# MerlinPCarson/WakeWord-Detection

Hardware: AMD Instinct MI355X
Metric: audio frames/sec (16 kHz, 40-mel, 10 ms hop) + FRR@0.5 FA/h (higher is better)
Workload: dtype f32; 1 GPU; CRNN forward, batch=256x1.5 s synthetic 16 kHz clips per GPU, PCM resident in HBM -> log-mel (fp64 FFT) -> 151x40 window -> encode+detect, fp32 MFMA; clips_per_gpu=256, samples_per_clip=24000, resident_input_batches_rotated=24, resident_input_bytes=294912000, pipelined_contexts=4, weights=reference tf_lite_models (shipped fp32 weights), parallelism=single GPU

## Files before the change

### wakeword-detection_amd/csrc/crnn.hip

```cpp
#include "stream_fe.h"
#include <algorithm>
#include <type_traits>

#include <cstdlib>

typedef float f32x4 __attribute__((ext_vector_type(4)));

struct win_addr {
  const int64_t *row;
  const int32_t *valid;
  int64_t row0;
  int hop;
  int valid_const;
  int64_t mel_rows;
};

__device__ __forceinline__ void window_span(const win_addr &wa, int w, int T, int64_t &row, int &valid) {
  if (wa.row && wa.valid) {
    const int64_t r = wa.row[w];
    const int v = wa.valid[w];
    row = r;
    valid = v;
  } else {
    row = wa.row ? wa.row[w] : wa.row0 + (int64_t)w * wa.hop;
// ... 132 lines not shown
  for (int ni = 0; ni < 2; ++ni) {
    const int gn = n0 + wc * 32 + ni * 16 + i16;
    const float bv = (gn < g.N) ? g.bias[gn] : 0.f;
#pragma unroll
    for (int r = 0; r < 4; ++r) {
      const int gm = m0 + wr * 16 + kk * 4 + r;
      if (gm < g.M && gn < g.N) g.C[(size_t)gm * g.N + gn] = acc[ni][r] + bv;
    }
  }
}

#define GR_H 32
#define GR_SEQ_LD 68
#define GR_GX_LD 196
#define GR_W1_LD 65

__device__ __forceinline__ float fast_sigmoid(float x) {
  return __builtin_amdgcn_rcpf(1.0f + __builtin_amdgcn_exp2f(-1.4426950408889634f * x));
}
__device__ __forceinline__ float fast_tanh(float x) {
  const float e = __builtin_amdgcn_exp2f(2.8853900817779268f * x);
  return __fmaf_rn(-2.0f, __builtin_amdgcn_rcpf(1.0f + e), 1.0f);
}
__device__ __forceinline__ float gru_candidate(float r, float hc, float xc) { return fast_tanh(__fmaf_rn(r, hc, xc)); }
__device__ __forceinline__ float gru_blend(float z, float h, float c) { return __fmaf_rn(z, h, __fmul_rn(__fsub_rn(1.0f, z), c)); }

__device__ __forceinline__ float swap_pair(float v) {
  return __int_as_float(__builtin_amdgcn_mov_dpp(__float_as_int(v), 0xB1, 0xF, 0xF, true));
}

typedef float f32x2 __attribute__((ext_vector_type(2)));

struct gru_w {
  f32x2 z[8], r[8], c[8];
  float bz, br, bc;
};

__device__ __forceinline__ void gru_load_w(gru_w &g, const float *wh, const float *bh, int dir, int unit, int half) {
  const float *base = wh + (size_t)dir * 3 * GR_H * GR_H;
#pragma unroll
  for (int q = 0; q < 4; ++q) {
    const float4 z = *(const float4 *)(base + (size_t)(0 * GR_H + unit) * GR_H + half * 16 + q * 4);
    const float4 r = *(const float4 *)(base + (size_t)(1 * GR_H + unit) * GR_H + half * 16 + q * 4);
    const float4 c = *(const float4 *)(base + (size_t)(2 * GR_H + unit) * GR_H + half * 16 + q * 4);
    g.z[2 * q] = (f32x2){z.x, z.y}; g.z[2 * q + 1] = (f32x2){z.z, z.w};
    g.r[2 * q] = (f32x2){r.x, r.y}; g.r[2 * q + 1] = (f32x2){r.z, r.w};
    g.c[2 * q] = (f32x2){c.x, c.y}; g.c[2 * q + 1] = (f32x2){c.z, c.w};
  }
  g.bz = half ? 0.f : bh[dir * 3 * GR_H + unit];
  g.br = half ? 0.f : bh[dir * 3 * GR_H + GR_H + unit];
  g.bc = half ? 0.f : bh[dir * 3 * GR_H + 2 * GR_H + unit];
}

template <bool PREFETCH>
__device__ __forceinline__ float gru_step(const gru_w &g, const float *hin, int half, float gz, float gr, float gc, float h_own,
                                          const float *gx_next, float &nz, float &nr, float &nc) {
  const float4 *hp = (const float4 *)(hin + half * 16);
  float4 hv[4];
  hv[0] = hp[0];
  __builtin_amdgcn_sched_barrier(0);
  hv[1] = hp[1];
  hv[2] = hp[2];
  hv[3] = hp[3];
  __builtin_amdgcn_sched_barrier(0);
  if (PREFETCH) {
    nz = gx_next[0];
    nr = gx_next[GR_H];
    nc = gx_next[2 * GR_H];
  }
  f32x2 az = {half ? 0.f : gz, g.bz}, ar = {half ? 0.f : gr, g.br}, ac = {0.f, g.bc};
  __builtin_amdgcn_sched_barrier(0);
#pragma unroll
  for (int q = 0; q < 4; ++q) {
    const f32x2 h0 = {hv[q].x, hv[q].y}, h1 = {hv[q].z, hv[q].w};
    az = __builtin_elementwise_fma(g.z[2 * q], h0, az); ar = __builtin_elementwise_fma(g.r[2 * q], h0, ar); ac = __builtin_elementwise_fma(g.c[2 * q], h0, ac);
    __builtin_amdgcn_sched_barrier(0);
    az = __builtin_elementwise_fma(g.z[2 * q + 1], h1, az); ar = __builtin_elementwise_fma(g.r[2 * q + 1], h1, ar); ac = __builtin_elementwise_fma(g.c[2 * q + 1], h1, ac);
    __builtin_amdgcn_sched_barrier(0);
  }
  float sz = az.x + az.y, sr = ar.x + ar.y, sc = ac.x + ac.y;
  sz += swap_pair(sz);
  sr += swap_pair(sr);
  sc += swap_pair(sc);
  const float z = fast_sigmoid(sz);
  const float r = fast_sigmoid(sr);
  return gru_blend(z, h_own, gru_candidate(r, sc, gc));
}

__device__ __forceinline__ void wsync_h() {
  asm volatile("" ::: "memory");
  __builtin_amdgcn_wave_barrier();
}

__device__ __forceinline__ void lds_barrier() {
  asm volatile("s_waitcnt lgkmcnt(0)\n\ts_barrier" ::: "memory");
}

__device__ __forceinline__ void wsync_g() {
  asm volatile("s_waitcnt lgkmcnt(0)" ::: "memory");
  __builtin_amdgcn_wave_barrier();
}

#define CLEAR_SEQ_H(seq1_, rows_, hb_, threads_)                                      \
  for (int i = tid; i < (rows_) * GR_SEQ_LD; i += (threads_)) (seq1_)[i] = 0.f;       \
  for (int i = tid; i < 2 * 2 * 2 * GR_H; i += (threads_)) (hb_)[i] = 0.f;

#define CV_LOAD_W(wreg_, wlast_, cb0_, cb1_, w4_, cbias_)                                            \
  _Pragma("unroll") for (int kb = 0; kb < CV_KB; ++kb)                                               \
    _Pragma("unroll") for (int n = 0; n < 2; ++n)                                                    \
      wreg_[kb][n] = *(const float4 *)((w4_) + ((size_t)(kb * 4 + kk) * 32 + n * 16 + j) * 4);       \
  _Pragma("unroll") for (int n = 0; n < 2; ++n)                                                      \
    wlast_[n] = (w4_)[((size_t)CV_QL * 32 + n * 16 + j) * 4 + kk];                                   \
  cb0_ = (cbias_)[j];                                                                                \
  cb1_ = (cbias_)[16 + j];
struct cv_a {
  float4 q[CV_KB];
  float last;
};
#define CV_LOAD_A(av_, abase_)                                                                       \
  _Pragma("unroll") for (int kb = 0; kb < CV_KB; ++kb) {                                             \
    const int k4 = kb * 16 + kk * 4;                                                                 \
    const int kf = k4 / CV_KT, kt = k4 - kf * CV_KT;                                                 \
    av_.q[kb] = *(const float4 *)((abase_) + kf * CV_LDT + kt);                                      \
  }                                                                                                  \
  av_.last = (abase_)[(CV_QL * 4 / CV_KT) * CV_LDT + CV_QL * 4 % CV_KT + kk];
#define CV_MFMA_KB(av_, kb_)                                                                         \
  acc0 = __builtin_amdgcn_mfma_f32_16x16x4f32(av_.q[kb_].x, wreg[kb_][0].x, acc0, 0, 0, 0);           \
  acc1 = __builtin_amdgcn_mfma_f32_16x16x4f32(av_.q[kb_].x, wreg[kb_][1].x, acc1, 0, 0, 0);           \
  acc0 = __builtin_amdgcn_mfma_f32_16x16x4f32(av_.q[kb_].y, wreg[kb_][0].y, acc0, 0, 0, 0);           \
  acc1 = __builtin_amdgcn_mfma_f32_16x16x4f32(av_.q[kb_].y, wreg[kb_][1].y, acc1, 0, 0, 0);           \
  acc0 = __builtin_amdgcn_mfma_f32_16x16x4f32(av_.q[kb_].z, wreg[kb_][0].z, acc0, 0, 0, 0);           \
  acc1 = __builtin_amdgcn_mfma_f32_16x16x4f32(av_.q[kb_].z, wreg[kb_][1].z, acc1, 0, 0, 0);           \
  acc0 = __builtin_amdgcn_mfma_f32_16x16x4f32(av_.q[kb_].w, wreg[kb_][0].w, acc0, 0, 0, 0);           \
  acc1 = __builtin_amdgcn_mfma_f32_16x16x4f32(av_.q[kb_].w, wreg[kb_][1].w, acc1, 0, 0, 0);
#define CV_MFMA_LAST(av_)                                                                            \
  acc0 = __builtin_amdgcn_mfma_f32_16x16x4f32(av_.last, wlast[0], acc0, 0, 0, 0);                     \
  acc1 = __builtin_amdgcn_mfma_f32_16x16x4f32(av_.last, wlast[1], acc1, 0, 0, 0);
#define CV_TILE_LOOP(NT_, ...)                                                                       \
  {                                                                                                  \
    cv_a av[2];                                                                                      \
    load_a(av[0], 0);                                                                                \
    _Pragma("unroll") for (int i = 0; i < NT_; ++i) {                                                \
      if (i + 1 < NT_) load_a(av[(i + 1) & 1], i + 1);                                               \
      __builtin_amdgcn_sched_barrier(0);                                                             \
      f32x4 acc0 = {cb0, cb0, cb0, cb0}, acc1 = {cb1, cb1, cb1, cb1};                                \
      CV_MFMA_KB(av[i & 1], 0) CV_MFMA_KB(av[i & 1], 1) CV_MFMA_KB(av[i & 1], 2)                     \
      __builtin_amdgcn_sched_barrier(0);                                                             \
      __VA_ARGS__                                                                                    \
      __builtin_amdgcn_sched_barrier(0);                                                             \
      CV_MFMA_KB(av[i & 1], 3) CV_MFMA_KB(av[i & 1], 4) CV_MFMA_KB(av[i & 1], 5) CV_MFMA_LAST(av[i & 1]) \
      prev0 = acc0;                                                                                  \
      prev1 = acc1;                                                                                  \
    }                                                                                                \
  }

#define PJ_KS_BYTES (4 * 192 * 16)
typedef const __attribute__((address_space(1))) char *pj_gptr;
typedef const __attribute__((address_space(1))) f32x4 *pj_gptr4;
__device__ __forceinline__ float4 pj_w_ld(pj_gptr4 p) {
  const f32x4 v = *p;
  return make_float4(v.x, v.y, v.z, v.w);
}
#define PJ_W_LANE(wx1s_)                                                                             \
  const pj_gptr wb_0 = (pj_gptr)(wx1s_);                                                             \
  unsigned wb_lane = (unsigned)((kk * 192 + wave * 48 + j) * 16);
#define PJ_W_KSTEP(wk_, ks_)                                                                         \
  pj_gptr wk_ = wb_0 + (size_t)(ks_) * PJ_KS_BYTES;                                                  \
  asm("" : "+s"(wk_));                                                                               \
// ... 24 lines not shown
    if (ks + 1 < 40) { __VA_ARGS__ }                                                                 \
    __builtin_amdgcn_sched_barrier(0);                                                               \
    const float4 *b = bq[ks % DEPTH_];                                                               \
    G16_(x) G3_(x) G16_(y) G3_(y) G16_(z) G3_(z) G16_(w) G3_(w)                                      \
    __builtin_amdgcn_sched_barrier(0);                                                               \
  }
#define PJ_REM_ROWS(rem_, bv_, ...)                                                                  \
  _Pragma("unroll") for (int i = 0; i < 3; ++i) {                                                    \
    float s3 = rem_[i];                                                                              \
    s3 += __shfl_xor(s3, 16);                                                                        \
    s3 += __shfl_xor(s3, 32);                                                                        \
    if (kk == 0) {                                                                                   \
      const float v = s3 + bv_;                                                                      \
      __VA_ARGS__                                                                                    \
    }                                                                                                \
  }

#define CF_THREADS 256
#define CF_FLD 648
#define CF_IMG_FLOATS (CV_ROWS * CV_LDT)
#define CF_FEAT_FLOATS (CV_OT * CF_FLD)
#define CF_SMEM_BYTES ((CF_IMG_FLOATS + CF_FEAT_FLOATS) * 4)
#define CF_NO_ROW (-0x40000000)
#define CF_FUSED_FEAT_ROWS 13
#define CF_FUSED_SMEM_BYTES ((CF_IMG_FLOATS + CF_FUSED_FEAT_ROWS * CF_FLD) * 4)
#define CF_ALIAS_ROWS0 24
#define CF_ALIAS_REM (CF_ALIAS_ROWS0 + 3 * CF_FLD)
static_assert((((CF_ALIAS_ROWS0 - CF_IMG_FLOATS) / 4 - 2 * 13) % 16 + 16) % 16 == 0 && CF_IMG_FLOATS % 4 == 0, "aliased rows off their bank slots");
static_assert(CV_OT - 16 == 3 && 16 - CF_FUSED_FEAT_ROWS == 3 && CF_ALIAS_REM + 20 * 96 <= 20 * GR_GX_LD ,
              "the aliased rows must lie under gx");
#define CF_GX 0
#define CF_SEQ (20 * GR_GX_LD)
#define CF_HB (CF_SEQ + 32 * GR_SEQ_LD)
#define CF_ENC (CF_HB + 2 * 2 * 2 * GR_H)
#define CF_HID (CF_ENC + 2 * GR_H)
#define CF_W2S (CF_HID + 2 * GR_H)
static_assert(CF_W2S + 8 * 64 <= CF_IMG_FLOATS, "post-conv LDS layout exceeds the image region");
static_assert(64 * GR_W1_LD <= CF_FEAT_FLOATS && 16 * 192 * 4 <= CF_FEAT_FLOATS, "feat region too small for its later tenants");
static_assert(64 * GR_W1_LD <= CF_FUSED_FEAT_ROWS * CF_FLD, "fused kernel's feat region too small for the head's first layer");

struct fused_args {
  const float *mel;
  win_addr wa;
  const float *w4;
  const float *cbias;
  const float *wx1s;
  const float *bx1;
  const float *wh1, *bh1;
  const float *wx2s;
  const float *bx2, *wh2, *bh2, *w1, *b1, *w2, *b2;
  float *enc;
  float *out;
  int T, NOUT, HEAD;
  long long *stamps;
  float *gx_out;
  const unsigned short *cwb;
  const unsigned short *wx1b;
  ww_tick_tag tag;
};

template <bool SEQ>
__device__ __forceinline__ float cf_recurrence(const gru_w &g, const float *gxs, float *hd, float *seq1, int dir, int unit, int half) {
  constexpr int H = GR_H, OT = CV_OT;
  const float *gxl = gxs + dir * 3 * H + unit;
  float h_own = 0.f;
  int t = dir ? OT - 1 : 0;
  float gz = gxl[t * GR_GX_LD], gr = gxl[t * GR_GX_LD + H], gc = gxl[t * GR_GX_LD + 2 * H];
  for (int s = 0; s < OT; ++s) {
    const int cur = s & 1;
    const int tn = dir ? (t > 0 ? t - 1 : 0) : (t + 1 < OT ? t + 1 : OT - 1);
    float nz, nr, nc;
    h_own = gru_step<true>(g, hd + cur * H, half, gz, gr, gc, h_own, gxl + tn * GR_GX_LD, nz, nr, nc);
    if (half == 0) {
      hd[(cur ^ 1) * H + unit] = h_own;
      if (SEQ) seq1[t * GR_SEQ_LD + dir * H + unit] = h_own;
    }
    wsync_h();
    gz = nz; gr = nr; gc = nc;
    t = tn;
  }
  return h_own;
}

#define CF_ROUND_L2(av_, rv_, b_, e_)                                                                  \
  acc[0] = __builtin_amdgcn_mfma_f32_16x16x4f32(av_.e_, b_[0].e_, acc[0], 0, 0, 0);                     \
  acc[1] = __builtin_amdgcn_mfma_f32_16x16x4f32(av_.e_, b_[1].e_, acc[1], 0, 0, 0);                     \
  acc[2] = __builtin_amdgcn_mfma_f32_16x16x4f32(av_.e_, b_[2].e_, acc[2], 0, 0, 0);                     \
  rem[0] = __builtin_amdgcn_mfma_f32_16x16x4f32(rv_.e_, b_[0].e_, rem[0], 0, 0, 0);                     \
  rem[1] = __builtin_amdgcn_mfma_f32_16x16x4f32(rv_.e_, b_[1].e_, rem[1], 0, 0, 0);                     \
  rem[2] = __builtin_amdgcn_mfma_f32_16x16x4f32(rv_.e_, b_[2].e_, rem[2], 0, 0, 0);

#define L2_LOAD_W(bq_, wx2s_, nt0_)                                                                  \
  _Pragma("unroll") for (int kb = 0; kb < 4; ++kb)                                                   \
    _Pragma("unroll") for (int n = 0; n < 3; ++n)                                                    \
      bq_[kb][n] = *(const float4 *)((wx2s_) + ((size_t)(kb * 4 + kk) * 192 + ((nt0_) + n) * 16 + j) * 4);
#define L2_LOAD_BIAS(bb_, bx2_, nt0_) \
  _Pragma("unroll") for (int n = 0; n < 3; ++n) bb_[n] = (bx2_)[((nt0_) + n) * 16 + j];
#define L2_PROJECT(bq_, bb_, rrow_, nt0_, ...)                                                       \
  {                                                                                                  \
    f32x4 acc[3] = {{0.f, 0.f, 0.f, 0.f}, {0.f, 0.f, 0.f, 0.f}, {0.f, 0.f, 0.f, 0.f}};               \
    f32x4 rem[3] = {{0.f, 0.f, 0.f, 0.f}, {0.f, 0.f, 0.f, 0.f}, {0.f, 0.f, 0.f, 0.f}};               \
    _Pragma("unroll") for (int kb = 0; kb < 4; ++kb) {                                               \
      const float4 av = *(const float4 *)(&seq1[j * GR_SEQ_LD + kb * 16 + kk * 4]);                  \
      const float4 rv = *(const float4 *)(&seq1[(rrow_) * GR_SEQ_LD + kb * 16 + kk * 4]);            \
      const float4 *b = bq_[kb];                                                                     \
      CF_ROUND_L2(av, rv, b, x) CF_ROUND_L2(av, rv, b, y) CF_ROUND_L2(av, rv, b, z) CF_ROUND_L2(av, rv, b, w) \
    }                                                                                                \
    __VA_ARGS__                                                                                      \
    _Pragma("unroll") for (int n = 0; n < 3; ++n) {                                                  \
      const int col = ((nt0_) + n) * 16 + j;                                                         \
      const float bb = bb_[n];                                                                       \
      _Pragma("unroll") for (int r = 0; r < 4; ++r) gxs[(kk * 4 + r) * GR_GX_LD + col] = acc[n][r] + bb; \
      if (kk == 0) {                                                                                 \
        _Pragma("unroll") for (int r = 0; r < 3; ++r) gxs[(16 + r) * GR_GX_LD + col] = rem[n][r] + bb; \
      }                                                                                              \
    }                                                                                                \
  }

__device__ __forceinline__ void cf_phases_d_to_g(const fused_args &a, float *img, float *feat, const gru_w &g, int w) {
  constexpr int H = GR_H;
  const int tid = threadIdx.x, lane = tid & 63, wave = tid >> 6;
  const int j = lane & 15, kk = lane >> 4;
  const int unit = lane >> 1, half = lane & 1, dir = wave & 1;
  float *gxs = img + CF_GX, *seq1 = img + CF_SEQ, *hb = img + CF_HB, *encs = img + CF_ENC, *hid = img + CF_HID, *w2s = img + CF_W2S;
  float4 bq2[4][3];
  L2_LOAD_W(bq2, a.wx2s, wave * 3)
  if (wave < 2) {
    __builtin_amdgcn_s_setprio(3);
    cf_recurrence<true>(g, gxs, hb + dir * 2 * H, seq1, dir, unit, half);
    __builtin_amdgcn_s_setprio(0);
  }
  __syncthreads();

  {
    float bb2[3];
    L2_LOAD_BIAS(bb2, a.bx2, wave * 3)
    __builtin_amdgcn_sched_barrier(0);
    L2_PROJECT(bq2, bb2, 16 + j, wave * 3, )
  }
  __syncthreads();

  float *w1s = feat;
  if (wave >= 2) {
    __builtin_amdgcn_s_setprio(3);
    const float h_last = cf_recurrence<false>(g, gxs, hb + (2 + dir) * 2 * H, nullptr, dir, unit, half);
    __builtin_amdgcn_s_setprio(0);
    if (half == 0) {
      encs[dir * H + unit] = h_last;
      if (a.enc) a.enc[(size_t)w * 2 * H + dir * H + unit] = h_last;
    }
  } else {
    for (int i = tid; i < 64 * 64; i += 128) w1s[(i >> 6) * GR_W1_LD + (i & 63)] = a.w1[i];
    for (int i = tid; i < a.NOUT * 64; i += 128) w2s[i] = a.w2[i];
  }
  __syncthreads();

  if (wave == 0) {
    const float b1v = a.b1[lane], b2v = a.b2[lane < a.NOUT ? lane : 0];
    __builtin_amdgcn_sched_barrier(0);
    float acc = 0.f;
#pragma unroll 16
    for (int k = 0; k < 2 * H; ++k) acc = fmaf(w1s[lane * GR_W1_LD + k], encs[k], acc);
    hid[lane] = fmaxf(acc + b1v, 0.f);
    wsync_g();
    float y = 0.f;
    if (lane < a.NOUT) {
      for (int k = 0; k < 2 * H; ++k) y = fmaf(w2s[lane * 64 + k], hid[k], y);
      y += b2v;
    }
    const float p = head_activation(y, lane, a.NOUT, a.HEAD);
    if (a.tag.slots) {
      if (lane == a.tag.pidx) tick_tag_store(a.tag, w, p);
    } else if (lane < a.NOUT) {
      a.out[(size_t)w * a.NOUT + lane] = p;
    }
  }
}

#define CF_STAMP(i_) \
  if (FRONT_ONLY && a.stamps && lane == 0) a.stamps[((size_t)blockIdx.x * 4 + wave) * 10 + (i_)] = __builtin_amdgcn_s_memtime();
__device__ __forceinline__ void cf_set_move(fused_args &a, long long off) {
  ww_set_move(a.w4, off); ww_set_move(a.cbias, off); ww_set_move(a.wx1s, off); ww_set_move(a.bx1, off);
  ww_set_move(a.wh1, off); ww_set_move(a.bh1, off); ww_set_move(a.wx2s, off); ww_set_move(a.bx2, off);
  ww_set_move(a.wh2, off); ww_set_move(a.bh2, off); ww_set_move(a.w1, off); ww_set_move(a.b1, off);
  ww_set_move(a.w2, off); ww_set_move(a.b2, off); ww_set_move(a.cwb, off); ww_set_move(a.wx1b, off);
}
template <bool FRONT_ONLY, bool SET = false>
__global__ __launch_bounds__(CF_THREADS, 2) void crnn_fused_kernel(fused_args a, ww_set_ref set) {
  if constexpr (SET) cf_set_move(a, ww_set_offset(set, blockIdx.x));
  extern __shared__ __align__(16) float cf_smem[];
  float *img = cf_smem, *feat = cf_smem + CF_IMG_FLOATS;
  constexpr int H = GR_H, OT = CV_OT;
  const int tid = threadIdx.x, lane = tid & 63, wave = tid >> 6;
  const int j = lane & 15, kk = lane >> 4;
  const int w = blockIdx.x;
  CF_STAMP(0)
  int64_t row;
  int valid;
  window_span(a.wa, w, a.T, row, valid);

  float4 wreg[CV_KB][2];
  float wlast[2], cb0, cb1;
  CV_LOAD_W(wreg, wlast, cb0, cb1, a.w4, a.cbias)

  int a_off[6], o_off[6][4];
  {
    constexpr int MAXV = 6;
    const float *src = a.mel + row * CV_NMEL;
    const int n = valid * CV_NMEL;
    const bool al16 = ((((uintptr_t)src) & 15) == 0);
    float4 stage[MAXV];
    if (n > 0)
      stage_loads(al16, [&](auto al) {
        constexpr bool AL = decltype(al)::value;
#pragma unroll
        for (int q = 0; q < MAXV; ++q) {
          const int i = (q * CF_THREADS + tid) * 4;
          stage[q] = ld_mel4<AL>(src + (i < n ? i : n - 4), true);
        }
      });
    LDS_CLEAR16(img, CF_IMG_FLOATS / 4, CF_THREADS)
// ... 644 lines not shown
  }
  __syncthreads();
  if (FRONT_ONLY) {
    float4 *dst = (float4 *)(a.gx_out + (size_t)w * OT * 6 * H);
    for (int q = tid; q < OT * 6 * H / 4; q += CF_THREADS) {
      const int e = q * 4, t = e / (6 * H), c = e - t * 6 * H;
      dst[q] = *(const float4 *)(&gxs[t * GR_GX_LD + c]);
    }
    return;
  }
  cf_phases_d_to_g(a, img, feat, g, w);
}

struct tail_args {
  const float *gx1;
  const float *wh1, *bh1;
  const float *wx2s;
  const float *bx2, *wh2, *bh2, *w1, *b1, *w2, *b2;
  float *enc, *out;
  int NOUT, HEAD;
  const float *gxI, *gxL, *gxR;
  int hop_g, eight_g;
  const int64_t *iI0;
  const float *wx2;
};
#define GT_SEQ (19 * GR_GX_LD)
#define GT_HB (GT_SEQ + 20 * GR_SEQ_LD)
#define GT_ENC (GT_HB + 2 * 2 * 2 * GR_H)
#define GT_HID (GT_ENC + 2 * GR_H)
#define GT_SMEM_FLOATS (GT_HID + 2 * GR_H)

__device__ __forceinline__ void gt_set_move(tail_args &a, const ww_set_ref &set, int slot) {
  const long long off = ww_set_offset(set, slot);
  ww_set_move(a.wh1, off); ww_set_move(a.bh1, off); ww_set_move(a.wx2s, off); ww_set_move(a.wx2, off); ww_set_move(a.bx2, off);
  ww_set_move(a.wh2, off); ww_set_move(a.bh2, off); ww_set_move(a.w1, off); ww_set_move(a.b1, off); ww_set_move(a.w2, off);
  ww_set_move(a.b2, off);
  const size_t nI = (size_t)set.aux[WW_SLIDE_AUX_NI], nW = (size_t)set.aux[WW_SLIDE_AUX_NW], W = (size_t)set.aux[WW_SLIDE_AUX_W];
  a.gxI += (size_t)slot * nI * 6 * GR_H;
  a.gxL += (size_t)slot * nW * 6 * GR_H;
  a.gxR += (size_t)slot * nW * 6 * GR_H;
  a.out += (size_t)slot * W * a.NOUT;
}

template <bool SET = false>
__global__ __launch_bounds__(128, 4) void gru_tail_kernel(tail_args a, ww_set_ref set) {
  if constexpr (SET) gt_set_move(a, set, blockIdx.y);
  constexpr int H = GR_H, OT = CV_OT;
  __shared__ __align__(16) float sm[GT_SMEM_FLOATS];
  float *gxs = sm, *seq1 = sm + GT_SEQ, *hb = sm + GT_HB, *encs = sm + GT_ENC, *hid = sm + GT_HID;
  const int tid = threadIdx.x, lane = tid & 63, dir = tid >> 6;
  const int j = lane & 15, kk = lane >> 4, unit = lane >> 1, half = lane & 1;
  const int w = blockIdx.x;
  gru_w g;
  gru_load_w(g, a.wh1, a.bh1, dir, unit, half);
  {
    constexpr int NQ = OT * 6 * H / 4, NS = (NQ + 127) / 128;
    int64_t i0w = (int64_t)w * a.hop_g;
    if (!a.gx1 && a.iI0) i0w = a.iI0[w];
    f32x4 st[NS];
#pragma unroll
    for (int s = 0; s < NS; ++s) {
      const int q = min(tid + 128 * s, NQ - 1), t = q / 48, c4 = q - t * 48;
      const float *row = a.gx1 ? a.gx1 + ((size_t)w * OT + t) * 6 * H
                       : t == 0 ? a.gxL + (size_t)w * 6 * H
                       : t == OT - 1 ? a.gxR + (size_t)w * 6 * H
                                     : a.gxI + ((size_t)i0w + (size_t)(t - 1) * a.eight_g) * 6 * H;
      st[s] = *(const f32x4 *)(row + c4 * 4);
    }
#pragma unroll
    for (int s = 0; s < NS; ++s) {
      const int q = tid + 128 * s, t = q / 48, c4 = q - t * 48;
      if (q < NQ) *(f32x4 *)(&gxs[t * GR_GX_LD + c4 * 4]) = st[s];
    }
  }
  CLEAR_SEQ_H(seq1, 20, hb, 128)
  __syncthreads();
  cf_recurrence<true>(g, gxs, hb + dir * 2 * H, seq1, dir, unit, half);
  __syncthreads();
#pragma unroll 1
  for (int pass = 0; pass < 2; ++pass) {
    const int nt0 = dir * 6 + pass * 3;
    float4 bq[4][3];
    L2_LOAD_W(bq, a.wx2s, nt0)
    float bb2[3];
    L2_LOAD_BIAS(bb2, a.bx2, nt0)
    L2_PROJECT(bq, bb2, j < 3 ? 16 + j : 19 , nt0, __syncthreads();)
  }
  gru_w g2;
  gru_load_w(g2, a.wh2, a.bh2, dir, unit, half);
  __syncthreads();
  const float h_last = cf_recurrence<false>(g2, gxs, hb + (2 + dir) * 2 * H, nullptr, dir, unit, half);
  if (half == 0) {
    encs[dir * H + unit] = h_last;
    if (a.enc) a.enc[(size_t)w * 2 * H + dir * H + unit] = h_last;
  }
  __syncthreads();
  if (dir == 0) {
    const float b1v = a.b1[lane], b2v = a.b2[lane < a.NOUT ? lane : 0];
    float acc = 0.f;
    const float4 *wr = (const float4 *)(a.w1 + (size_t)lane * 2 * H);
#pragma unroll
    for (int q = 0; q < 16; ++q) {
      const float4 wv = wr[q];
      const float4 ev = *(const float4 *)(&encs[q * 4]);
      acc = fmaf(wv.x, ev.x, acc); acc = fmaf(wv.y, ev.y, acc);
      acc = fmaf(wv.z, ev.z, acc); acc = fmaf(wv.w, ev.w, acc);
    }
    hid[lane] = fmaxf(acc + b1v, 0.f);
    wsync_g();
    float y = 0.f;
    if (lane < a.NOUT) {
      for (int k = 0; k < 2 * H; ++k) y = fmaf(a.w2[lane * 64 + k], hid[k], y);
      y += b2v;
    }
    const float p = head_activation(y, lane, a.NOUT, a.HEAD);
    if (lane < a.NOUT) a.out[(size_t)w * a.NOUT + lane] = p;
  }
}

#define GT16_LD 36
#define GT16_ELD 68
#define GT16_SMEM_BYTES ((2 * 2 * 16 * GT16_LD + 2 * 6 * 2 * 64 * 4) * 4)
struct tail16_args {
  tail_args t;
  float *seq;
  int nw;
};

template <bool SET = false>
__global__ __launch_bounds__(128, 2) void gru_tail16_kernel(tail16_args aa, ww_set_ref set) {
  if constexpr (SET) {
    gt_set_move(aa.t, set, blockIdx.y);
    aa.seq += (size_t)blockIdx.y * (size_t)((aa.nw + 15) / 16) * CV_OT * 16 * 2 * GR_H;
  }
  constexpr int H = GR_H, OT = CV_OT;
  const tail_args &a = aa.t;
  extern __shared__ __align__(16) float sm16[];
  float (*hs)[2][16 * GT16_LD] = (float (*)[2][16 * GT16_LD])sm16;
  float *encs = sm16 + 2 * 2 * 16 * GT16_LD, *hid = encs + 16 * GT16_ELD;
  static_assert(2 * 16 * GT16_ELD <= 2 * 6 * 2 * 64 * 4, "enc / hid rows do not fit the weight pages");
  const int tid = threadIdx.x, lane = tid & 63, dir = tid >> 6;
  const int c = lane & 15, g = lane >> 4;
  float4 *whl = (float4 *)(sm16 + 2 * 2 * 16 * GT16_LD) + (size_t)dir * 6 * 2 * 64 + lane;
  const int w0 = blockIdx.x * 16;
  float *seq = aa.seq + (size_t)blockIdx.x * OT * 16 * 2 * H;

  int wi[4];
  int64_t i0[4];
#pragma unroll
  for (int r = 0; r < 4; ++r) wi[r] = min(w0 + 4 * g + r, aa.nw - 1);
  if (!a.gx1 && a.iI0) {
#pragma unroll
    for (int r = 0; r < 4; ++r) i0[r] = a.iI0[wi[r]];
  } else {
#pragma unroll
    for (int r = 0; r < 4; ++r) i0[r] = a.gx1 ? 0 : (int64_t)wi[r] * a.hop_g;
  }
  auto gx_row = [&](int r, int t) -> const float * {
    if (a.gx1) return a.gx1 + ((size_t)wi[r] * OT + t) * 6 * H;
    if (t == 0) return a.gxL + (size_t)wi[r] * 6 * H;
    if (t == OT - 1) return a.gxR + (size_t)wi[r] * 6 * H;
    return a.gxI + (size_t)(i0[r] + (int64_t)(t - 1) * a.eight_g) * 6 * H;
  };
#define GT16_POS(u_) (8 * (((u_) >> 1) & 3) + 4 * ((u_) >> 4) + 2 * (((u_) >> 3) & 1) + ((u_) & 1))
  float bh[6];
  auto load_wh = [&](const float *whp, const float *bhp) {
#pragma unroll
    for (int nt = 0; nt < 6; ++nt) {
      const int row = (nt >> 1) * H + (nt & 1) * 16 + c;
// ... 124 lines not shown
#define GT16_PROJ(q_, kb_)                                                                           \
  _Pragma("unroll") for (int nt = 0; nt < 6; ++nt) gx2[nt] = __builtin_amdgcn_mfma_f32_16x16x4f32(q_.x, wx[nt][4 * kb_ + 0], gx2[nt], 0, 0, 0); \
  _Pragma("unroll") for (int nt = 0; nt < 6; ++nt) gx2[nt] = __builtin_amdgcn_mfma_f32_16x16x4f32(q_.y, wx[nt][4 * kb_ + 1], gx2[nt], 0, 0, 0); \
  _Pragma("unroll") for (int nt = 0; nt < 6; ++nt) gx2[nt] = __builtin_amdgcn_mfma_f32_16x16x4f32(q_.z, wx[nt][4 * kb_ + 2], gx2[nt], 0, 0, 0); \
  _Pragma("unroll") for (int nt = 0; nt < 6; ++nt) gx2[nt] = __builtin_amdgcn_mfma_f32_16x16x4f32(q_.w, wx[nt][4 * kb_ + 3], gx2[nt], 0, 0, 0);
    GT16_PROJ(q0, 0)
    GT16_PROJ(q1, 1)
    GT16_PROJ(q2, 2)
    GT16_PROJ(q3, 3)
#undef GT16_PROJ
#pragma unroll
    for (int nt = 0; nt < 6; ++nt) gx2[nt] += (f32x4){bx[nt], bx[nt], bx[nt], bx[nt]};
  };
  project(dir ? OT - 1 : 0);
  __syncthreads();
#pragma unroll 1
  for (int s = 0; s < OT; ++s) {
    const int t = dir ? OT - 1 - s : s, cur = s & 1;
    f32x4 pre[6];
    const f32x4 zero4 = {0.f, 0.f, 0.f, 0.f};
    if (s > 0) {
      const float4 *hp = (const float4 *)(&hs[dir][cur][c * GT16_LD + 8 * g]);
      const float4 a0 = hp[0], a1 = hp[1];
      const float ha[8] = {a0.x, a0.y, a0.z, a0.w, a1.x, a1.y, a1.z, a1.w};
      GT16_PRE_ALL(gx2)
    } else {
      GT16_PRE_FIRST(gx2)
    }
#pragma unroll
    for (int uh = 0; uh < 2; ++uh)
#pragma unroll
      for (int r = 0; r < 4; ++r) {
        const float z = fast_sigmoid(pre[uh][r]);
        const float rr = fast_sigmoid(pre[2 + uh][r]);
        const float hn = gru_blend(z, h_own[r][uh], gru_candidate(rr, pre[4 + uh][r], gx2[4 + uh][r]));
        h_own[r][uh] = hn;
        hs[dir][cur ^ 1][(4 * g + r) * GT16_LD + (uh ? pos1 : pos0)] = hn;
      }
    if (s + 1 < OT) project(dir ? t - 1 : t + 1);
    wsync_h();
  }
  __syncthreads();
#pragma unroll
  for (int uh = 0; uh < 2; ++uh)
#pragma unroll
    for (int r = 0; r < 4; ++r) {
      encs[(4 * g + r) * GT16_ELD + dir * H + uh * 16 + c] = h_own[r][uh];
      if (a.enc && w0 + 4 * g + r < aa.nw) a.enc[(size_t)(w0 + 4 * g + r) * 2 * H + dir * H + uh * 16 + c] = h_own[r][uh];
    }
  __syncthreads();

  {
    float4 w1r[16];
    const float4 *wr = (const float4 *)(a.w1 + (size_t)lane * 2 * H);
#pragma unroll
    for (int q = 0; q < 16; ++q) w1r[q] = wr[q];
    const float b1v = a.b1[lane];
#pragma unroll 1
    for (int wq = dir * 8; wq < dir * 8 + 8; ++wq) {
      float acc = 0.f;
#pragma unroll
      for (int q = 0; q < 16; ++q) {
        const float4 ev = *(const float4 *)(&encs[wq * GT16_ELD + q * 4]);
        acc = fmaf(w1r[q].x, ev.x, acc); acc = fmaf(w1r[q].y, ev.y, acc);
        acc = fmaf(w1r[q].z, ev.z, acc); acc = fmaf(w1r[q].w, ev.w, acc);
      }
      hid[wq * GT16_ELD + lane] = fmaxf(acc + b1v, 0.f);
    }
  }
  __syncthreads();
  {
    const int wq = tid >> 3, o = tid & 7;
    float y = 0.f;
    if (o < a.NOUT) {
      for (int k = 0; k < 2 * H; ++k) y = fmaf(a.w2[o * 64 + k], hid[wq * GT16_ELD + k], y);
      y += a.b2[o];
    }
    const float p = head_activation(y, o, a.NOUT, a.HEAD);
    if (o < a.NOUT && w0 + wq < aa.nw) a.out[(size_t)(w0 + wq) * a.NOUT + o] = p;
  }
}


#undef CF_ROUND_L2
#undef L2_PROJECT
#undef PJ_KLOOP
#undef PJ_ROWS16
#undef PJ_ROWS3
#undef PJ_NO_ROWS
#undef CV_TILE_LOOP
#undef CV_MFMA_KB
#undef CV_MFMA_LAST
#undef GT16_PRE_ALL
#undef GT16_PRE_FIRST
#undef GT16_POS

__global__ __launch_bounds__(64) void crnn_detect_kernel(const float *enc, const float *w1, const float *b1, const float *w2,
                                                         const float *b2, float *out, int NOUT, int HEAD) {
  __shared__ float e[64], hid[64];
  const int lane = threadIdx.x, w = blockIdx.x;
  e[lane] = enc[(size_t)w * 64 + lane];
  __syncthreads();
  float acc = 0.f;
  for (int k = 0; k < 64; ++k) acc = fmaf(w1[lane * 64 + k], e[k], acc);
  hid[lane] = fmaxf(acc + b1[lane], 0.f);
  __syncthreads();
  float y = 0.f;
  if (lane < NOUT) {
    for (int k = 0; k < 64; ++k) y = fmaf(w2[lane * 64 + k], hid[k], y);
    y += b2[lane];
  }
  const float p = head_activation(y, lane, NOUT, HEAD);
  if (lane < NOUT) out[(size_t)w * NOUT + lane] = p;
}

int ww_k_crnn_detect(ww_ctx *ctx, const ww_model *m, const float *d_enc, int nw, float *d_out) {
  if (nw <= 0) return WW_OK;
  const ww_crnn_dev &c = m->crnn;
  ww_launch_scope scope(ctx, "crnn_detect_kernel");
  hipLaunchKernelGGL(crnn_detect_kernel, dim3(nw), dim3(64), 0, ctx->stream, d_enc, c.w1, c.b1, c.w2, c.b2, d_out, c.NOUT, c.HEAD);
  WW_HIP(ctx, hipGetLastError());
  return WW_OK;
}

struct convg_args {
  const float *mel;
  win_addr wa;
  const float *wt;
  const float *bias;
  float *feat;
  int n_mel, T, C, KF, KT, SF, ST, PF, PT, OF, OT, FEATP;
};

__global__ __launch_bounds__(256) void conv_generic_kernel(convg_args a) {
  extern __shared__ __align__(16) float cg_win[];
  const int tid = threadIdx.x, w = blockIdx.x;
  int64_t row;
  int valid;
  window_span(a.wa, w, a.T, row, valid);
  const float *src = a.mel + row * a.n_mel;
  for (int i = tid; i < a.T * a.n_mel; i += 256) cg_win[i] = i < valid * a.n_mel ? src[i] : 0.f;
  __syncthreads();
  float *dst = a.feat + (size_t)w * a.OT * a.FEATP;
  const int feat_w = a.OF * a.C;
  for (int o = tid; o < a.OT * a.FEATP; o += 256) {
    const int t = o / a.FEATP, col = o - t * a.FEATP;
    float v = 0.f;
    if (col < feat_w) {
      const int f = col / a.C, c = col - f * a.C;
      float acc = 0.f;
      for (int kf = 0; kf < a.KF; ++kf) {
        const int im = f * a.SF - a.PF + kf;
        if (im < 0 || im >= a.n_mel) continue;
        for (int kt = 0; kt < a.KT; ++kt) {
          const int it = t * a.ST - a.PT + kt;
          if (it < 0 || it >= a.T) continue;
          acc = fmaf(cg_win[it * a.n_mel + im], a.wt[(size_t)(kf * a.KT + kt) * a.C + c], acc);
        }
      }
      v = fmaxf(acc + a.bias[c], 0.f);
    }
    dst[o] = v;
  }
}

struct grug_args {
  const float *gx;
// ... 354 lines not shown
```

Before: 914.8 million audio frames/s.

## Use 4x4x1 MFMA for remainder rows and split GRU sigmoid across lane pairs

The layer-2 input projection previously computed the 3 leftover time rows with full 16x16x4 MFMAs, which wasted most of the tile. These rows now go through 4x4x1f32 MFMAs with broadcast control bits, and their weights are prefetched per lane with a lag/lookahead software pipeline interleaved with the main tiles. Separately, the GRU step now evaluates one sigmoid per lane of each lane pair and exchanges the result with swap_pair, halving transcendental work at the cost of an extra cross-lane swap. The change adds extra global weight loads and more complex scheduling, and may raise register pressure.

```diff
diff --git a/wakeword-detection_amd/csrc/crnn.hip b/wakeword-detection_amd/csrc/crnn.hip
--- a/wakeword-detection_amd/csrc/crnn.hip
+++ b/wakeword-detection_amd/csrc/crnn.hip
@@ -238,8 +238,10 @@
   sz += swap_pair(sz);
   sr += swap_pair(sr);
   sc += swap_pair(sc);
-  const float z = fast_sigmoid(sz);
-  const float r = fast_sigmoid(sr);
+  const float own = fast_sigmoid(half ? sz : sr);
+  const float other = swap_pair(own);
+  const float z = half ? own : other;
+  const float r = half ? other : own;
   return gru_blend(z, h_own, gru_candidate(r, sc, gc));
 }
 
@@ -430,38 +432,70 @@
   return h_own;
 }
 
-#define CF_ROUND_L2(av_, rv_, b_, e_)                                                                  \
+#define L2_REM_COL(nt0_) ((nt0_) * 16 + (l2_lane < 48 ? l2_lane : l2_lane - 16))
+#define L2_REM_LANE(nt0_)                                                                            \
+  int l2_lane = lane;                                                                                \
+  asm volatile("" : "+v"(l2_lane));  \
+  unsigned wr_lane = (unsigned)(L2_REM_COL(nt0_) * 16);
+#define L2_REM_LOAD_W(wq_, wx2s_, kb_)                                                               \
+  _Pragma("unroll") for (int q = 0; q < 4; ++q) {                                                    \
+    pj_gptr wr_k = (pj_gptr)(wx2s_) + (size_t)((kb_) * 4 + q) * (192 * 16);                          \
+    asm("" : "+s"(wr_k));                                                                            \
+    asm("" : "+v"(wr_lane));                                                                         \
+    wq_[q] = pj_w_ld((pj_gptr4)(wr_k + wr_lane));                                                    \
+  }
+#define L2_ROUND_MAIN(av_, b_, e_)                                                                     \
   acc[0] = __builtin_amdgcn_mfma_f32_16x16x4f32(av_.e_, b_[0].e_, acc[0], 0, 0, 0);                     \
   acc[1] = __builtin_amdgcn_mfma_f32_16x16x4f32(av_.e_, b_[1].e_, acc[1], 0, 0, 0);                     \
-  acc[2] = __builtin_amdgcn_mfma_f32_16x16x4f32(av_.e_, b_[2].e_, acc[2], 0, 0, 0);                     \
-  rem[0] = __builtin_amdgcn_mfma_f32_16x16x4f32(rv_.e_, b_[0].e_, rem[0], 0, 0, 0);                     \
-  rem[1] = __builtin_amdgcn_mfma_f32_16x16x4f32(rv_.e_, b_[1].e_, rem[1], 0, 0, 0);                     \
-  rem[2] = __builtin_amdgcn_mfma_f32_16x16x4f32(rv_.e_, b_[2].e_, rem[2], 0, 0, 0);
+  acc[2] = __builtin_amdgcn_mfma_f32_16x16x4f32(av_.e_, b_[2].e_, acc[2], 0, 0, 0);
+#define L2_ROUND_REM(ra_, wq_, e_, ei_)                                                                \
+  rem = __builtin_amdgcn_mfma_f32_4x4x1f32(ra_, wq_[0].e_, rem, 4, 0 + ei_, 0);                         \
+  rem = __builtin_amdgcn_mfma_f32_4x4x1f32(ra_, wq_[1].e_, rem, 4, 4 + ei_, 0);                         \
+  rem = __builtin_amdgcn_mfma_f32_4x4x1f32(ra_, wq_[2].e_, rem, 4, 8 + ei_, 0);                         \
+  rem = __builtin_amdgcn_mfma_f32_4x4x1f32(ra_, wq_[3].e_, rem, 4, 12 + ei_, 0);
+#define L2_ROUND(LAG_, e_, ei_)                                                                      \
+  if (kb < 4) { L2_ROUND_MAIN(av, b, e_) }                                                           \
+  if (kb >= LAG_) { L2_ROUND_REM(ra, wk, e_, ei_) }
 
 #define L2_LOAD_W(bq_, wx2s_, nt0_)                                                                  \
   _Pragma("unroll") for (int kb = 0; kb < 4; ++kb)                                                   \
     _Pragma("unroll") for (int n = 0; n < 3; ++n)                                                    \
       bq_[kb][n] = *(const float4 *)((wx2s_) + ((size_t)(kb * 4 + kk) * 192 + ((nt0_) + n) * 16 + j) * 4);
-#define L2_LOAD_BIAS(bb_, bx2_, nt0_) \
-  _Pragma("unroll") for (int n = 0; n < 3; ++n) bb_[n] = (bx2_)[((nt0_) + n) * 16 + j];
-#define L2_PROJECT(bq_, bb_, rrow_, nt0_, ...)                                                       \
+#define L2_LOAD_BIAS(bb_, bx2_, nt0_)                                                                \
+  _Pragma("unroll") for (int n = 0; n < 3; ++n) bb_[n] = (bx2_)[((nt0_) + n) * 16 + j];              \
+  bb_[3] = (bx2_)[L2_REM_COL(nt0_)];
+#define L2_PROJECT(LAG_, AHEAD_, bq_, wq0_, wx2s_, bb_, nt0_, ...)                                   \
   {                                                                                                  \
     f32x4 acc[3] = {{0.f, 0.f, 0.f, 0.f}, {0.f, 0.f, 0.f, 0.f}, {0.f, 0.f, 0.f, 0.f}};               \
-    f32x4 rem[3] = {{0.f, 0.f, 0.f, 0.f}, {0.f, 0.f, 0.f, 0.f}, {0.f, 0.f, 0.f, 0.f}};               \
-    _Pragma("unroll") for (int kb = 0; kb < 4; ++kb) {                                               \
-      const float4 av = *(const float4 *)(&seq1[j * GR_SEQ_LD + kb * 16 + kk * 4]);                  \
-      const float4 rv = *(const float4 *)(&seq1[(rrow_) * GR_SEQ_LD + kb * 16 + kk * 4]);            \
-      const float4 *b = bq_[kb];                                                                     \
-      CF_ROUND_L2(av, rv, b, x) CF_ROUND_L2(av, rv, b, y) CF_ROUND_L2(av, rv, b, z) CF_ROUND_L2(av, rv, b, w) \
+    f32x4 rem = {0.f, 0.f, 0.f, 0.f};                                                                \
+    const float *rp = &seq1[(16 + (l2_lane & 3)) * GR_SEQ_LD + (l2_lane >> 2)];                      \
+    float4 wq[4][4];                                                                                 \
+    _Pragma("unroll") for (int q = 0; q < 4; ++q) wq[0][q] = wq0_[q];                                \
+    float4 avq[2];     \
+    float raq[2];                                                                                    \
+    avq[0] = *(const float4 *)(&seq1[j * GR_SEQ_LD + kk * 4]);                                       \
+    if (LAG_ == 0) raq[0] = rp[0];                                                                   \
+    _Pragma("unroll") for (int kb = 0; kb < 4 + LAG_; ++kb) {                                        \
+      const int c = kb - LAG_;                                               \
+      if (c + AHEAD_ > 0 && c + AHEAD_ < 4) { L2_REM_LOAD_W(wq[c + AHEAD_], wx2s_, c + AHEAD_) }     \
+      if (kb + 1 < 4) avq[(kb + 1) & 1] = *(const float4 *)(&seq1[j * GR_SEQ_LD + (kb + 1) * 16 + kk * 4]); \
+      if (c + 1 >= 0 && c + 1 < 4) raq[(c + 1) & 1] = rp[(c + 1) * 16];                              \
+      const float4 av = avq[kb & 1];                                                                 \
+      const float ra = raq[c & 1];                                                                   \
+      __builtin_amdgcn_sched_barrier(0);                                                             \
+      const float4 *b = bq_[kb & 3];                                                                 \
+      const float4 *wk = wq[c & 3];                                                                  \
+      L2_ROUND(LAG_, x, 0) L2_ROUND(LAG_, y, 1) L2_ROUND(LAG_, z, 2) L2_ROUND(LAG_, w, 3)            \
+      __builtin_amdgcn_sched_barrier(0);                                                             \
     }                                                                                                \
     __VA_ARGS__                                                                                      \
     _Pragma("unroll") for (int n = 0; n < 3; ++n) {                                                  \
       const int col = ((nt0_) + n) * 16 + j;                                                         \
       const float bb = bb_[n];                                                                       \
       _Pragma("unroll") for (int r = 0; r < 4; ++r) gxs[(kk * 4 + r) * GR_GX_LD + col] = acc[n][r] + bb; \
-      if (kk == 0) {                                                                                 \
-        _Pragma("unroll") for (int r = 0; r < 3; ++r) gxs[(16 + r) * GR_GX_LD + col] = rem[n][r] + bb; \
-      }                                                                                              \
+    }                                                                                                \
+    if (l2_lane < 48) {                                                                              \
+      _Pragma("unroll") for (int r = 0; r < 3; ++r) gxs[(16 + r) * GR_GX_LD + (nt0_) * 16 + l2_lane] = rem[r] + bb_[3]; \
     }                                                                                                \
   }
 
@@ -478,13 +512,17 @@
     cf_recurrence<true>(g, gxs, hb + dir * 2 * H, seq1, dir, unit, half);
     __builtin_amdgcn_s_setprio(0);
   }
-  __syncthreads();
-
-  {
-    float bb2[3];
+  float4 wq2[4];
+  L2_REM_LANE(wave * 3)
+  L2_REM_LOAD_W(wq2, a.wx2s, 0)
+  __builtin_amdgcn_sched_barrier(0);
+  lds_barrier();
+
+  {
+    float bb2[4];
     L2_LOAD_BIAS(bb2, a.bx2, wave * 3)
     __builtin_amdgcn_sched_barrier(0);
-    L2_PROJECT(bq2, bb2, 16 + j, wave * 3, )
+    L2_PROJECT(1, 1, bq2, wq2, a.wx2s, bb2, wave * 3, )
   }
   __syncthreads();
 
@@ -1295,9 +1333,12 @@
     const int nt0 = dir * 6 + pass * 3;
     float4 bq[4][3];
     L2_LOAD_W(bq, a.wx2s, nt0)
-    float bb2[3];
+    float4 wq0[4];
+    L2_REM_LANE(nt0)
+    L2_REM_LOAD_W(wq0, a.wx2s, 0)
+    float bb2[4];
     L2_LOAD_BIAS(bb2, a.bx2, nt0)
-    L2_PROJECT(bq, bb2, j < 3 ? 16 + j : 19 , nt0, __syncthreads();)
+    L2_PROJECT(4, 3, bq, wq0, a.wx2s, bb2, nt0, __syncthreads();)
   }
   gru_w g2;
   gru_load_w(g2, a.wh2, a.bh2, dir, unit, half);
@@ -1588,7 +1629,9 @@
 }
 
 
-#undef CF_ROUND_L2
+#undef L2_ROUND
+#undef L2_ROUND_MAIN
+#undef L2_ROUND_REM
 #undef L2_PROJECT
 #undef PJ_KLOOP
 #undef PJ_ROWS16
```

Result: no change. 923.2 million audio frames/s (median of 6 runs) (+0.9%).
